# davxy/ark-vrf

Hardware: NVIDIA B200
Metric: bandersnatch_thin_vrf_batch_verified_proofs_per_sec (higher is better)
Workload: dtype u32

## Files before the change

__graft_entry__.py:

```python
import os
import subprocess
import sys

ROOT = os.path.dirname(os.path.abspath(__file__))
CSRC = os.path.join(ROOT, "ark_vrf_b200", "csrc")
LIB = os.path.join(ROOT, "ark_vrf_b200", "libavrf_gpu.so")
NVCC_FLAGS = ["-gencode", "arch=compute_100a,code=sm_100a", "-O3", "-lineinfo", "-std=c++17",
              "-Xcompiler", "-fPIC", "-shared"]


def _newer(target, sources):
    if not os.path.exists(target):
        return False
    t = os.path.getmtime(target)
    return all(os.path.getmtime(s) <= t for s in sources)


def build() -> None:
    srcs = [os.path.join(CSRC, f) for f in sorted(os.listdir(CSRC)) if f.endswith((".cu", ".cuh", ".h", ".cpp", ".inl"))]
    srcs.append(os.path.join(ROOT, "include", "avrf.h"))
    if not _newer(LIB, srcs):
        nvcc = os.environ.get("NVCC", "/usr/local/cuda/bin/nvcc")
        tmp = LIB + ".tmp"
        cmd = [nvcc] + NVCC_FLAGS + ["-o", tmp, os.path.join(CSRC, "avrf_gpu.cu"), os.path.join(CSRC, "mbsha512.cpp"),
                                   os.path.join(CSRC, "hostutil.cpp"),
                                   "-lcrypto", "-lpthread"]
        print("[build]", " ".join(cmd), flush=True)
        if os.path.exists(LIB):
            os.remove(LIB)
        subprocess.check_call(cmd)
        os.replace(tmp, LIB)
    emu_src = os.path.join(ROOT, "tests", "hostemu", "hostemu.cpp")
    emu_lib = os.path.join(ROOT, "tests", "hostemu", "libhostemu.so")
    if not _newer(emu_lib, srcs + [emu_src]):
        subprocess.check_call(["g++", "-O2", "-shared", "-fPIC", "-Wno-unknown-pragmas", "-o", emu_lib, emu_src])
    pl_src = os.path.join(ROOT, "tools", "push_loop.cpp")
    pl_lib = os.path.join(ROOT, "tools", "libavrf_pushloop.so")
    hdrs = [os.path.join(ROOT, "include", "avrf.h"), os.path.join(ROOT, "include", "avrf.hpp")]
    if os.path.exists(pl_src) and not _newer(pl_lib, hdrs + [pl_src, LIB]):
        pkg = os.path.join(ROOT, "ark_vrf_b200")
        subprocess.check_call(["g++", "-std=c++17", "-O2", "-shared", "-fPIC", "-I", os.path.join(ROOT, "include"), pl_src,
                               "-o", pl_lib, "-L", pkg, "-l:libavrf_gpu.so", "-Wl,-rpath," + pkg])
    mk = os.path.join(ROOT, "oracle", "Makefile")
    if os.path.exists(mk):
        subprocess.check_call(["make", "-s", "-C", os.path.join(ROOT, "oracle")])
    sys.path.insert(0, ROOT)
    import ark_vrf_b200
    ark_vrf_b200.load()


def smoke() -> None:
    sys.path.insert(0, ROOT)
    sys.path.insert(0, os.path.join(ROOT, "tests"))
    import ark_vrf_b200 as av
    from ark_vrf_b200 import synth
    from oracle import pyref as o
    av.load().avrf_init(0)
    sid, S, n = 0, o.BANDERSNATCH, 64
# ... 27 lines not shown
```

ark_vrf_b200/csrc/avrf_gpu.cu:

```cuda
#include <cstdlib>
#include <map>
#include <memory>
#include <new>
#include <vector>

#include "host_common.h"
#include "hostutil.h"
#include "feeders.cuh"
#include "verify_one.cuh"
#include "microbench.cuh"

using namespace avrf;

constexpr size_t PREP_CHUNK = 148 * 4 * 128;
constexpr size_t STAGE_CHUNK = PREP_CHUNK / 2;

struct PushStage {
  PinBuf pk, r, s, ios, ad, io_off, ad_off;
  size_t n = 0, nio = 0, nad = 0, cap_io = 0, cap_ad = 0;
  cudaEvent_t free_ev = nullptr;
  bool inflight = false;
};

struct avrf_batch {
  int device = 0;
  uint32_t suite = 0, fmt = 0, weights_mode = AVRF_WEIGHTS_REFERENCE;
  uint32_t scheme = 0;
  uint64_t n = 0, n_ios = 0, ad_bytes = 0;
  bool prepared = false;
  bool have_seed = false;
  bool want_taps = false;
  uint8_t seed[64];
  uint64_t first_index = 0;
  std::vector<uint64_t> segs;
  bool segs_dirty = false;
  DevBuf pk, r, s, ios, io_off, ad_off, ad;
  DevBuf ok, sb;
  PushStage stage[2];
  int cur = 0;
  std::vector<uint8_t> h_pk, h_r, h_s, h_ios, h_ad;
  std::vector<uint32_t> h_io_off{0}, h_ad_off{0};
  DevBuf dig_w, rank_w;
  DevBuf pts, cs, z, renc, digits, hist, cursor, offs, toff, btot, totals, entries, tasks, task_out, chunk_out, wsum,
      partial, gpart, flags, w_tap, scalars_tap, segs_dev;
  PinBuf h_cs, h_small;
  std::vector<cudaEvent_t> prep_ev;
  size_t prep_ev_chunks = 0;
  bool eager = true;
  std::unique_ptr<Hasher> hasher;
  Hasher* ext_hasher = nullptr;
  MbSha512* mb = nullptr;
  bool blocking = false;
  cudaEvent_t sync_ev = nullptr;
  uint64_t hashed = 0;
  uint64_t push_launches = 0;
  cudaStream_t st = nullptr, st_copy = nullptr, st_h2d = nullptr, st_prep = nullptr;
  ShardSlot* remote_slot = nullptr;
  bool inflight = false;
  bool inflight_did_prepare = false;
  int32_t early_status = -1;
  cudaEvent_t done_ev = nullptr;
  cudaEvent_t gate_ev = nullptr;
  cudaEvent_t h2d_gate_ev = nullptr;
  std::chrono::steady_clock::time_point t_verify0;
  cudaEvent_t ev[10] = {};
  avrf_timings tm = {};
};
// ... 30 lines not shown
  return CC_HOST[suite].suite_id;
}

static int finish_inflight(avrf_batch* b);

static int enter(avrf_batch* b) {
  if (!b) return fail(AVRF_ERR_ARG, "null batch");
  int rc = bind_device(b->device);
  if (rc) return rc;
  return b->inflight ? finish_inflight(b) : 0;
}
#define ENTER(b) do { int rc__ = enter(b); if (rc__) return rc__; } while (0)

static int quiesce(avrf_batch* b) {
  for (cudaStream_t q : {b->st_h2d, b->st_prep, b->st_copy, b->st}) CK(hsync(b, q));
  return 0;
}
static int grow(avrf_batch* b, DevBuf& buf, size_t bytes, size_t keep) {
  if (bytes <= buf.cap) return 0;
  int rc = quiesce(b);
  return rc ? rc : buf.reserve(bytes, keep, b->st);
}

static Hasher* hasher_of(avrf_batch* b) {
  if (b->ext_hasher) return b->ext_hasher;
  if (!b->hasher) {
    b->hasher.reset(new (std::nothrow) Hasher(b->device));
    if (b->hasher && b->mb) b->hasher->use_multibuffer(b->mb);
  }
  return b->hasher.get();
}

struct H2cScratch { DevBuf u01, den, scr; };
struct FeedPool {
  std::mutex mu;
  DevBuf b[12];
  H2cScratch w;
};
static FeedPool g_feed[AVRF_MAX_DEV];
static void feed_pool_release(int dev) {
  FeedPool& fp = g_feed[dev];
  std::lock_guard<std::mutex> lk(fp.mu);
  for (DevBuf& d : fp.b) d.release();
  fp.w.u01.release(); fp.w.den.release(); fp.w.scr.release();
}

// ... 114 lines not shown
  if (!b) return;
  bind_device(b->device);
  if (b->inflight) finish_inflight(b);
  b->hasher.reset();
  if (b->done_ev) cudaEventDestroy(b->done_ev);
  if (b->gate_ev) {
    MsmGate& g = g_gate[b->device];
    std::lock_guard<std::mutex> lk(g.mu);
    if (g.tail == b->gate_ev) g.tail = nullptr;
    cudaStreamSynchronize(b->st);
    cudaEventDestroy(b->gate_ev);
  }
  if (b->h2d_gate_ev) {
    MsmGate& g = g_h2d_gate[b->device];
    std::lock_guard<std::mutex> lk(g.mu);
    if (g.tail == b->h2d_gate_ev) g.tail = nullptr;
    cudaStreamSynchronize(b->st_h2d);
    cudaEventDestroy(b->h2d_gate_ev);
  }
  for (cudaStream_t q : {b->st, b->st_copy, b->st_h2d, b->st_prep}) if (q) cudaStreamSynchronize(q);
  DevBuf* bufs[] = {&b->ok, &b->sb, &b->pk, &b->r, &b->s, &b->ios, &b->io_off, &b->ad_off, &b->ad, &b->pts, &b->cs, &b->z, &b->renc,
                    &b->dig_w, &b->rank_w, &b->digits, &b->hist, &b->cursor, &b->offs, &b->toff, &b->btot, &b->totals, &b->entries, &b->tasks,
                    &b->task_out, &b->chunk_out, &b->wsum, &b->partial, &b->gpart, &b->flags, &b->w_tap, &b->scalars_tap,
                    &b->segs_dev};
  for (DevBuf* d : bufs) d->release();
  for (auto& e : b->ev) if (e) cudaEventDestroy(e);
  for (auto& e : b->prep_ev) cudaEventDestroy(e);
  for (auto& sg : b->stage) if (sg.free_ev) cudaEventDestroy(sg.free_ev);
  if (b->sync_ev) cudaEventDestroy(b->sync_ev);
  for (cudaStream_t q : {b->st, b->st_copy, b->st_h2d, b->st_prep}) if (q) cudaStreamDestroy(q);
  delete b;
}

int avrf_thin_batch_clear(avrf_batch* b) {
  ENTER(b);
  if (b->hasher) b->hasher->drain();
  for (auto& sg : b->stage) {
    if (sg.inflight) { CK(cudaEventSynchronize(sg.free_ev)); sg.inflight = false; }
    sg.n = sg.nio = sg.nad = 0;
  }
  b->n = b->n_ios = b->ad_bytes = 0;
  b->prepared = b->have_seed = false;
  b->hashed = 0;
  b->push_launches = 0;
  b->prep_ev_chunks = 0;
  b->segs.clear();
  b->segs_dirty = true;
// ... 166 lines not shown
      CK(cudaMemcpyAsync(b->sb.as<uint8_t>() + 32 * n0, sb, 32 * n, cudaMemcpyHostToDevice, b->st));
    }
    if (add_ios) CK(cudaMemcpyAsync(b->ios.as<uint8_t>() + 128 * i0, ios, 128 * add_ios, cudaMemcpyDefault, b->st));
    if (add_ad) CK(cudaMemcpyAsync(b->ad.as<uint8_t>() + a0, ad_blob, add_ad, cudaMemcpyDefault, b->st));
    if (consumed) CK(cudaEventRecord(consumed, b->st));
    b->n += n;
    b->n_ios += add_ios;
    b->ad_bytes += add_ad;
    b->prepared = b->have_seed = false;
    b->hashed = 0;
    b->prep_ev_chunks = 0;
    return 0;
  }
  Hasher* hs = hasher_of(b);
  if (!hs) return fail(AVRF_ERR_NOMEM, "hasher");
  size_t np_new = ped ? 5 * (n0 + n) + 2 : 2 * (n0 + n) + 2 * (i0 + add_ios) + 1;
  size_t np_old = n0 ? (ped ? 5 * n0 : 2 * n0 + 2 * i0) : 0;
  if ((rc = b->flags.reserve(64))) return rc;
  if ((rc = b->h_small.reserve(4096))) return rc;
  if ((rc = grow(b, b->pts, sizeof(BaseRec) * np_new, sizeof(BaseRec) * np_old))) return rc;
  if ((rc = grow(b, b->cs, stride * (n0 + n) + 64, stride * n0))) return rc;
  if ((rc = grow(b, b->z, 16 * (i0 + add_ios) + 16, 16 * i0))) return rc;
  if ((rc = grow(b, b->renc, 32 * (n0 + n) + 32, 32 * n0))) return rc;
  if (n0 == 0) {
    if (!b->ext_hasher) {
      size_t sl;
      const unsigned char* sid = suite_id_of(b->suite, &sl);
      unsigned char prefix[40];
      memcpy(prefix, sid, sl);
      prefix[sl] = DOM_BATCH;
      if ((rc = hs->begin(prefix, sl + 1))) return rc;
    }
    CK(cudaMemsetAsync(b->flags.p, 0, 64, b->st_prep));
  }
  if ((rc = hs->reserve_stage(std::max(stride * std::min<size_t>(n, 16 * PREP_CHUNK) + 64, stage_chunks * (stride * PREP_CHUNK + 64))))) return rc;
  size_t nch = (n + PREP_CHUNK - 1) / PREP_CHUNK;
  EventPool evs;
  cudaEvent_t off_ev = evs.make();
  if (!off_ev) return fail(AVRF_ERR_CUDA, "cudaEventCreate");
  CK(cudaEventRecord(off_ev, b->st_prep));
  CK(cudaStreamWaitEvent(b->st_h2d, off_ev, 0));
  PrepArgs a;
  PedPrepArgs pa;
  if (ped) {
    pa.pkcom = b->pk.as<Affine>(); pa.r = b->r.as<Affine>(); pa.ok = b->ok.as<Affine>(); pa.s = b->s.as<Fe>();
    pa.sb = b->sb.as<Fe>(); pa.ios = b->ios.as<Affine>(); pa.io_off = b->io_off.as<uint32_t>();
// ... 20 lines not shown
    CK(cudaMemcpyAsync(b->pk.as<uint8_t>() + 64 * (n0 + c0), pk + 64 * c0, 64 * cnt, cudaMemcpyDefault, b->st_h2d));
    CK(cudaMemcpyAsync(b->r.as<uint8_t>() + 64 * (n0 + c0), r + 64 * c0, 64 * cnt, cudaMemcpyDefault, b->st_h2d));
    CK(cudaMemcpyAsync(b->s.as<uint8_t>() + 32 * (n0 + c0), s + 32 * c0, 32 * cnt, cudaMemcpyDefault, b->st_h2d));
    if (ped) {
      CK(cudaMemcpyAsync(b->ok.as<uint8_t>() + 64 * (n0 + c0), ok + 64 * c0, 64 * cnt, cudaMemcpyDefault, b->st_h2d));
      CK(cudaMemcpyAsync(b->sb.as<uint8_t>() + 32 * (n0 + c0), sb + 32 * c0, 32 * cnt, cudaMemcpyDefault, b->st_h2d));
    }
    if (q1 > q0) CK(cudaMemcpyAsync(b->ios.as<uint8_t>() + 128 * (i0 + q0), ios + 128 * q0, 128 * (q1 - q0), cudaMemcpyDefault, b->st_h2d));
    if (d1 > d0) CK(cudaMemcpyAsync(b->ad.as<uint8_t>() + a0 + d0, ad_blob + d0, d1 - d0, cudaMemcpyDefault, b->st_h2d));
    CK(cudaEventRecord(h2d_ev, b->st_h2d));
    CK(cudaStreamWaitEvent(b->st_prep, h2d_ev, 0));
    if (ped) {
      pa.first = (uint32_t)(n0 + c0);
      pa.n = (uint32_t)(n0 + c1);
      DISPATCH(b->suite, (k_prepare_ped<S><<<cdiv(cnt, 128), 128, 0, b->st_prep>>>(pa)));
    } else {
      a.first = (uint32_t)(n0 + c0);
      a.n = (uint32_t)(n0 + c1);
      DISPATCH(b->suite, (k_prepare<S><<<cdiv(cnt, 128), 128, 0, b->st_prep>>>(a)));
    }
    LAUNCHED("k_prepare");
    CK(cudaEventRecord(prep_ev, b->st_prep));
    CK(cudaStreamWaitEvent(b->st_copy, prep_ev, 0));
    uint8_t* dst = hs->stage(stride * cnt);
    if (!dst) return fail(AVRF_ERR_NOMEM, "pinned staging");
    CK(cudaMemcpyAsync(dst, b->cs.as<uint8_t>() + stride * (n0 + c0), stride * cnt, cudaMemcpyDeviceToHost, b->st_copy));
    CK(cudaEventCreateWithFlags(&d2h_ev, cudaEventDisableTiming | cudaEventBlockingSync));
    CK(cudaEventRecord(d2h_ev, b->st_copy));
    hs->enqueue(d2h_ev, dst, stride * cnt);
  }
  CK(cudaEventRecord(b->h2d_gate_ev, b->st_h2d));
  hgate.tail = b->h2d_gate_ev;
  hgate_lock.unlock();
  if (consumed) CK(cudaEventRecord(consumed, b->st_prep));
  b->n += n;
  b->n_ios += add_ios;
  b->ad_bytes += add_ad;
  b->hashed = b->n;
  b->prepared = true;
  b->have_seed = false;
  b->prep_ev_chunks = 0;
  b->push_launches += nch;
  return 0;
}

static int stage_reserve(PushStage& sg, size_t cap_io, size_t cap_ad) {
  int rc;
  if ((rc = sg.pk.reserve(64 * PREP_CHUNK)) || (rc = sg.r.reserve(64 * PREP_CHUNK)) || (rc = sg.s.reserve(32 * PREP_CHUNK)) ||
      (rc = sg.io_off.reserve(4 * (PREP_CHUNK + 1))) || (rc = sg.ad_off.reserve(4 * (PREP_CHUNK + 1))))
    return rc;
  if (cap_io > sg.cap_io) { if ((rc = sg.ios.reserve(128 * cap_io, 128 * sg.nio))) return rc; sg.cap_io = cap_io; }
  if (cap_ad > sg.cap_ad) { if ((rc = sg.ad.reserve(cap_ad, sg.nad))) return rc; sg.cap_ad = cap_ad; }
  if (!sg.free_ev) CK(cudaEventCreateWithFlags(&sg.free_ev, cudaEventDisableTiming));
  return 0;
}

static int flush_stage(avrf_batch* b) {
  PushStage& sg = b->stage[b->cur];
  if (sg.n == 0) return 0;
  { int rc0 = bind_device(b->device); if (rc0) return rc0; }
  stage_fence();
  int rc = push_many_impl(b, sg.n, sg.pk.as<uint8_t>(), sg.ios.as<uint8_t>(), sg.io_off.as<uint32_t>(), sg.ad.as<uint8_t>(),
                          sg.ad_off.as<uint32_t>(), sg.r.as<uint8_t>(), sg.s.as<uint8_t>(), nullptr, nullptr, sg.free_ev,
                          sg.n == STAGE_CHUNK ? 4 : 0);
  if (rc) return rc;
// ... 71 lines not shown
  if ((io_offsets[n] && !ios) || (ad_offsets[n] && !ad_blob)) return fail(AVRF_ERR_ARG, "null argument");
  ENTER(b);
  int rc = flush_pending(b);
  if (rc) return rc;
  rc = push_many_impl(b, n, pk, ios, io_offsets, ad_blob, ad_offsets, r, s);
  if (rc) return rc;
  CK(hsync(b, b->st_h2d));
  CK(hsync(b, b->prepared ? b->st_prep : b->st));
  return 0;
}

int avrf_thin_batch_prepare(avrf_batch* b, int32_t* invalid) {
  ENTER(b);
  int rc = flush_pending(b);
  if (rc) return rc;
  if ((rc = b->flags.reserve(64))) return rc;
  if ((rc = b->h_small.reserve(4096))) return rc;
  if (!b->prepared) {
    size_t np = npoints_of(b);
    if ((rc = grow(b, b->pts, sizeof(BaseRec) * np, 0))) return rc;
    if ((rc = grow(b, b->cs, cs_stride(b) * b->n + 64, 0))) return rc;
    if ((rc = grow(b, b->z, 16 * b->n_ios + 16, 0))) return rc;
    if ((rc = grow(b, b->renc, 32 * b->n + 32, 0))) return rc;
    CK(cudaMemsetAsync(b->flags.p, 0, 64, b->st));
    size_t nch = (b->n + PREP_CHUNK - 1) / PREP_CHUNK;
    while (b->prep_ev.size() < nch) {
      cudaEvent_t e;
      CK(cudaEventCreateWithFlags(&e, cudaEventDisableTiming));
      b->prep_ev.push_back(e);
    }
    PedPrepArgs pa;
    PrepArgs ta;
    if (b->scheme == 1) {
      pa.pkcom = b->pk.as<Affine>(); pa.r = b->r.as<Affine>(); pa.ok = b->ok.as<Affine>(); pa.s = b->s.as<Fe>();
      pa.sb = b->sb.as<Fe>(); pa.ios = b->ios.as<Affine>(); pa.io_off = b->io_off.as<uint32_t>();
      pa.ad_off = b->ad_off.as<uint32_t>(); pa.ad = b->ad.as<uint8_t>(); pa.pts = b->pts.as<BaseRec>();
      pa.cs = b->cs.as<uint32_t>(); pa.flags = b->flags.as<int>(); pa.n = (uint32_t)b->n;
      pa.canonical = b->fmt == AVRF_FMT_CANONICAL;
    } else {
      ta.pk = b->pk.as<Affine>(); ta.r = b->r.as<Affine>(); ta.s = b->s.as<Fe>(); ta.ios = b->ios.as<Affine>();
      ta.io_off = b->io_off.as<uint32_t>(); ta.ad_off = b->ad_off.as<uint32_t>(); ta.ad = b->ad.as<uint8_t>();
      ta.pts = b->pts.as<BaseRec>(); ta.cs = b->cs.as<uint32_t>(); ta.z = b->z.as<uint32_t>();
      ta.renc = b->renc.as<uint32_t>(); ta.flags = b->flags.as<int>(); ta.n = (uint32_t)b->n;
      ta.canonical = b->fmt == AVRF_FMT_CANONICAL;
    }
    cudaStream_t ps = b->st_prep;
    {
      cudaEvent_t e;
      CK(cudaEventCreateWithFlags(&e, cudaEventDisableTiming));
      cudaEventRecord(e, b->st);
      cudaStreamWaitEvent(ps, e, 0);
      cudaEventDestroy(e);
    }
    if (nch) cudaEventRecord(b->ev[0], ps);
    for (size_t c = 0; c < nch; c++) {
      size_t cnt = std::min((size_t)PREP_CHUNK, (size_t)b->n - c * PREP_CHUNK);
      if (b->scheme == 1) {
        pa.first = (uint32_t)(c * PREP_CHUNK);
        DISPATCH(b->suite, (k_prepare_ped<S><<<cdiv(cnt, 128), 128, 0, ps>>>(pa)));
      } else {
        ta.first = (uint32_t)(c * PREP_CHUNK);
        DISPATCH(b->suite, (k_prepare<S><<<cdiv(cnt, 128), 128, 0, ps>>>(ta)));
      }
      LAUNCHED(b->scheme == 1 ? "k_prepare_ped" : "k_prepare");
      CK(cudaEventRecord(b->prep_ev[c], ps));
    }
    if (nch) {
      cudaEventRecord(b->ev[1], ps);
      cudaStreamWaitEvent(b->st, b->ev[1], 0);
      b->tm.kernel_launches = nch;
    }
    b->prep_ev_chunks = nch;
    b->prepared = true;
    b->have_seed = false;
  } else {
    cudaEvent_t e;
    CK(cudaEventCreateWithFlags(&e, cudaEventDisableTiming));
    cudaEventRecord(e, b->st_prep);
    cudaStreamWaitEvent(b->st, e, 0);
    cudaEventDestroy(e);
  }
  if (invalid) {
    CK(cudaMemcpyAsync(b->h_small.p, b->flags.p, 8, cudaMemcpyDeviceToHost, b->st));
    CK(hsync(b, b->st));
    int fl = reinterpret_cast<int*>(b->h_small.p)[0];
    if (fl & 2) return fail(AVRF_ERR_ARG, "an input coordinate or scalar is not below its modulus (not a field element)");
    *invalid = fl & 1;
  }
  return 0;
}

int avrf_thin_batch_cs_stream(avrf_batch* b, uint8_t* out) {
  if (!b || !out) return fail(AVRF_ERR_ARG, "null argument");
// ... 156 lines not shown
  if (b->want_taps) {
    if ((rc = b->w_tap.reserve(32 * b->n + 32))) return rc;
    if ((rc = b->scalars_tap.reserve(32 * np))) return rc;
  }
  cudaStream_t st = b->st;
  if (!b->gate_ev) CK(cudaEventCreateWithFlags(&b->gate_ev, cudaEventDisableTiming));
  if (b->segs.size() > 2 && b->segs_dirty) {
    if ((rc = b->segs_dev.reserve(8 * b->segs.size()))) return rc;
    CK(cudaMemcpyAsync(b->segs_dev.p, b->segs.data(), 8 * b->segs.size(), cudaMemcpyHostToDevice, st));
    CK(hsync(b, st));
    b->segs_dirty = false;
  }
  MsmGate& gate = g_gate[b->device];
  std::unique_lock<std::mutex> gate_lock(gate.mu);
  if (gate.tail && gate.tail != b->gate_ev) CK(cudaStreamWaitEvent(st, gate.tail, 0));
  CK(cudaMemsetAsync(b->hist.p, 0, 4 * MSM_NBINS, st));

  ScalArgs a;
  a.cs = b->cs.as<uint32_t>(); a.z = b->z.as<uint32_t>(); a.io_off = b->io_off.as<uint32_t>();
  a.digits = b->digits.as<uint4>(); a.hist = b->hist.as<uint32_t>(); a.gpart = b->gpart.as<uint32_t>();
  a.ranks = b->cursor.as<uint4>();
  a.w_tap = b->want_taps ? b->w_tap.as<uint32_t>() : nullptr;
  a.scalars_tap = b->want_taps ? b->scalars_tap.as<Fe>() : nullptr;
  seed_to_words(a.seed, seed);
  a.first_index = b->segs.size() == 2 ? b->segs[1] : first_index;
  a.segs = b->segs.size() > 2 ? b->segs_dev.as<uint64_t>() : nullptr;
  a.nseg = (uint32_t)(b->segs.size() / 2);
  b->first_index = first_index;
  a.n = (uint32_t)b->n;
  uint32_t* hist = b->hist.as<uint32_t>();
  uint32_t* offs = b->offs.as<uint32_t>();
  uint32_t* nzr = b->toff.as<uint32_t>();
  uint32_t* totals = b->totals.as<uint32_t>();
  Ext* slots = b->task_out.as<Ext>();
  cudaEventRecord(b->ev[2], st);
  if (b->scheme == 1) {
    PedScalArgs pa;
    pa.cs = a.cs; pa.digits = a.digits; pa.ranks = a.ranks; pa.hist = a.hist; pa.gpart = a.gpart;
    pa.w_tap = b->want_taps ? b->w_tap.as<uint32_t>() : nullptr;
    pa.scalars_tap = a.scalars_tap; pa.seed = a.seed; pa.first_index = a.first_index; pa.segs = a.segs; pa.nseg = a.nseg;
    pa.n = a.n;
    DISPATCH(b->suite, (k_scalars_ped<S><<<nblk, 128, 0, st>>>(pa)));
    LAUNCHED("k_scalars_ped");
    DISPATCH(b->suite, (k_gscalar_ped<S><<<1, 32, 0, st>>>(a.gpart, nblk, a.digits, a.ranks, a.hist, a.scalars_tap,
                                                            b->pts.as<BaseRec>(), np - 2)));
    LAUNCHED("k_gscalar_ped");
  } else {
    DISPATCH(b->suite, (k_scalars<S><<<nblk, 128, 0, st>>>(a)));
    LAUNCHED("k_scalars");
    DISPATCH(b->suite, (k_gscalar<S><<<1, 256, 0, st>>>(a.gpart, nblk, a.digits, a.ranks, a.hist, a.scalars_tap,
                                                         b->pts.as<BaseRec>(), np - 1)));
    LAUNCHED("k_gscalar");
  }
  cudaEventRecord(b->ev[3], st);
  k_scan_local<<<MSM_NBINS / 1024, 1024, 0, st>>>(hist, offs, nzr, b->btot.as<uint32_t>());
  LAUNCHED("k_scan_local");
  k_scan_totals<<<1, 512, 0, st>>>(b->btot.as<uint32_t>(), totals, offs);
  LAUNCHED("k_scan_totals");
  k_scan_add<<<MSM_NBINS / 1024, 1024, 0, st>>>(offs, nzr, b->btot.as<uint32_t>());
  LAUNCHED("k_scan_add");
  if (np >= (1u << 18)) {
    static std::once_flag smem_once[AVRF_MAX_DEV];
    std::call_once(smem_once[b->device], [] {
      cudaFuncSetAttribute(k_scatter_window, cudaFuncAttributeMaxDynamicSharedMemorySize, 4 * MSM_NBUCKET);
    });
    k_sort_transpose<<<cdiv(np, SORT_TP), SORT_TP, 0, st>>>(b->digits.as<uint4>(), b->cursor.as<uint4>(), np, np_pad,
                                                            b->dig_w.as<uint16_t>(), b->rank_w.as<uint32_t>());
    LAUNCHED("k_sort_transpose");
    k_scatter_window<<<dim3(37, MSM_NWIN), 1024, 4 * MSM_NBUCKET, st>>>(b->dig_w.as<uint16_t>(), b->rank_w.as<uint32_t>(), np, np_pad,
                                                                         offs, b->entries.as<uint32_t>());
    LAUNCHED("k_scatter_window");
  } else {
// ... 7 lines not shown
  ac.pts = b->pts.as<BaseRec>(); ac.slots = slots; ac.nthr = acc_nthr;
  if (b->suite == 0) k_accumulate<0, 4><<<acc_blocks, 128, 0, st>>>(ac);
  else if (b->suite == 2) k_accumulate<2, 4><<<acc_blocks, 128, 0, st>>>(ac);
  else k_accumulate<1, 5><<<acc_blocks, 128, 0, st>>>(ac);
  LAUNCHED("k_accumulate");
  cudaEventRecord(b->ev[5], st);
  CK(cudaEventRecord(b->gate_ev, st));
  gate.tail = b->gate_ev;
  gate_lock.unlock();
  DISPATCH(b->suite, (k_combine<S><<<MSM_NBINS / 128, 128, 0, st>>>(hist, offs, nzr, slots, acc_nthr, totals,
                                                                    b->tasks.as<uint32_t>())));
  LAUNCHED("k_combine");
  DISPATCH(b->suite, (k_combine_big<S><<<64, 256, 0, st>>>(hist, offs, nzr, slots, acc_nthr, totals,
                                                           b->tasks.as<uint32_t>())));
  LAUNCHED("k_combine_big");
  DISPATCH(b->suite, (k_bucket_reduce<S><<<MSM_NWIN * MSM_NCHUNK / 128, 128, 0, st>>>(hist, offs, nzr, acc_nthr, totals, slots,
                                                                                      b->chunk_out.as<Ext>())));
  LAUNCHED("k_bucket_reduce");
  DISPATCH(b->suite, (k_window_sum<S><<<MSM_NWIN, 256, 0, st>>>(b->chunk_out.as<Ext>(), b->wsum.as<Ext>())));
  LAUNCHED("k_window_sum");
  DISPATCH(b->suite, (k_fold<S><<<1, 32, 0, st>>>(b->wsum.as<Ext>(), b->partial.as<Ext>(), b->flags.as<int>(), b->remote_slot)));
  LAUNCHED("k_fold");
  cudaEventRecord(b->ev[6], st);
  b->tm.kernel_launches += 12;
  b->tm.n_points = np;
  return 0;
}

static void collect_timings(avrf_batch* b, bool with_prepare) {
  float ms = 0;
  if (with_prepare && cudaEventElapsedTime(&ms, b->ev[0], b->ev[1]) == cudaSuccess) b->tm.prepare_ms = ms;
  if (cudaEventElapsedTime(&ms, b->ev[2], b->ev[3]) == cudaSuccess) b->tm.scalars_ms = ms;
  if (cudaEventElapsedTime(&ms, b->ev[3], b->ev[4]) == cudaSuccess) b->tm.sort_ms = ms;
  if (cudaEventElapsedTime(&ms, b->ev[4], b->ev[5]) == cudaSuccess) b->tm.accumulate_ms = ms;
  if (cudaEventElapsedTime(&ms, b->ev[5], b->ev[6]) == cudaSuccess) b->tm.reduce_ms = ms;
  (void)cudaGetLastError();
}

extern "C" {

int avrf_thin_seed_dev(uint32_t suite, const void* cs_stream_dev, uint64_t n_items, uint8_t seed[64]) {
  if (suite > 2 || !seed || (n_items && !cs_stream_dev)) return fail(AVRF_ERR_ARG, "bad argument");
  NEED_DEVICE();
  std::lock_guard<std::mutex> lock(g_pin_mu);
  return seed_of_device_stream(gs(), gc(), suite, (const uint8_t*)cs_stream_dev, 64 * n_items, g_pin_stream[g_device.load()], seed, nullptr);
}

// ... 264 lines not shown
```

ark_vrf_b200/csrc/msm.cuh:

```cuda
#pragma once
#include "thin.cuh"

namespace avrf {

constexpr int MSM_WBITS = 16;
constexpr int MSM_NWIN = 16;
constexpr int MSM_NBUCKET = 1 << (MSM_WBITS - 1);
constexpr int MSM_NBINS = MSM_NWIN * MSM_NBUCKET;
constexpr int MSM_CHUNK = 16;
constexpr int MSM_NCHUNK = MSM_NBUCKET / MSM_CHUNK;

struct Seed64 { uint64_t w[8]; };

#ifdef __CUDACC__

__device__ __forceinline__ void load_affinek(AffineK& q, const BaseRec* p) {
  const uint4* s = reinterpret_cast<const uint4*>(p);
  uint4 a0 = __ldg(s + 0), a1 = __ldg(s + 1), a2 = __ldg(s + 2), a3 = __ldg(s + 3), a4 = __ldg(s + 4), a5 = __ldg(s + 5);
  q.x.v[0] = a0.x; q.x.v[1] = a0.y; q.x.v[2] = a0.z; q.x.v[3] = a0.w;
  q.x.v[4] = a1.x; q.x.v[5] = a1.y; q.x.v[6] = a1.z; q.x.v[7] = a1.w;
  q.y.v[0] = a2.x; q.y.v[1] = a2.y; q.y.v[2] = a2.z; q.y.v[3] = a2.w;
  q.y.v[4] = a3.x; q.y.v[5] = a3.y; q.y.v[6] = a3.z; q.y.v[7] = a3.w;
  q.k.v[0] = a4.x; q.k.v[1] = a4.y; q.k.v[2] = a4.z; q.k.v[3] = a4.w;
  q.k.v[4] = a5.x; q.k.v[5] = a5.y; q.k.v[6] = a5.z; q.k.v[7] = a5.w;
// ... 1 lines not shown

__device__ __forceinline__ void store_fe(Fe* dst, const Fe& a) {
  uint4* d = reinterpret_cast<uint4*>(dst);
  d[0] = make_uint4(a.v[0], a.v[1], a.v[2], a.v[3]);
  d[1] = make_uint4(a.v[4], a.v[5], a.v[6], a.v[7]);
}

__device__ __forceinline__ void load_fe(Fe& a, const Fe* src) {
  const uint4* s = reinterpret_cast<const uint4*>(src);
  uint4 lo = s[0], hi = s[1];
  a.v[0] = lo.x; a.v[1] = lo.y; a.v[2] = lo.z; a.v[3] = lo.w;
  a.v[4] = hi.x; a.v[5] = hi.y; a.v[6] = hi.z; a.v[7] = hi.w;
}

__device__ __forceinline__ void store_ext(Ext* dst, const Ext& p) {
  store_fe(&dst->x, p.x); store_fe(&dst->y, p.y); store_fe(&dst->z, p.z); store_fe(&dst->t, p.t);
}

__device__ __forceinline__ void load_ext(Ext& p, const Ext* src) {
  load_fe(p.x, &src->x); load_fe(p.y, &src->y); load_fe(p.z, &src->z); load_fe(p.t, &src->t);
}

__device__ __forceinline__ void emit_scalar(uint4* digits, uint32_t* hist, uint4* ranks, Fe* scalars_tap, size_t point,
                                            const Fe& k) {
  int32_t dg[16];
  recode_signed16(dg, k);
  uint32_t pk[8];
#pragma unroll
  for (int i = 0; i < 8; i++) pk[i] = ((uint32_t)dg[2 * i] & 0xffffu) | ((uint32_t)dg[2 * i + 1] << 16);
  digits[2 * point] = make_uint4(pk[0], pk[1], pk[2], pk[3]);
  digits[2 * point + 1] = make_uint4(pk[4], pk[5], pk[6], pk[7]);
  uint32_t rk[16];
#pragma unroll
  for (int i = 0; i < 16; i++) {
    int32_t d = dg[i];
    rk[i] = 0;
    if (d != 0) {
      uint32_t mag = d < 0 ? (uint32_t)(-d) : (uint32_t)d;
      rk[i] = atomicAdd(&hist[i * MSM_NBUCKET + mag - 1], 1u);
    }
  }
#pragma unroll
  for (int i = 0; i < 4; i++) ranks[4 * point + i] = make_uint4(rk[4 * i], rk[4 * i + 1], rk[4 * i + 2], rk[4 * i + 3]);
  if (scalars_tap) store_fe(&scalars_tap[point], k);
}

struct ScalArgs {
  const uint32_t* cs;
  const uint32_t* z;
  const uint32_t* io_off;
  uint4* digits;
  uint4* ranks;
  uint32_t* hist;
  uint32_t* gpart;
  uint32_t* w_tap;
  Fe* scalars_tap;
  Seed64 seed;
  uint64_t first_index;
  const uint64_t* segs;
  uint32_t nseg;
  uint32_t n;
};

__device__ __forceinline__ uint64_t global_index(uint64_t first_index, const uint64_t* segs, uint32_t nseg, uint32_t j) {
  if (nseg <= 1) return first_index + j;
  uint32_t lo = 0, hi = nseg;
  while (hi - lo > 1) {
    uint32_t mid = (lo + hi) >> 1;
    if (segs[2 * mid] <= j) lo = mid;
    else hi = mid;
  }
  return segs[2 * lo + 1] + (j - segs[2 * lo]);
}

__device__ __forceinline__ void add10(uint32_t* a, const uint32_t* b) {
  a[0] = add_cc(a[0], b[0]);
#pragma unroll
  for (int i = 1; i < 9; i++) a[i] = addc_cc(a[i], b[i]);
  a[9] = addc(a[9], b[9]);
}

constexpr uint32_t SCAL_PER_THREAD = 1;
template <int S>
__global__ void __launch_bounds__(128) k_scalars(ScalArgs a) {
  constexpr int FR = SuiteT<S>::FR;
// ... 8 lines not shown
    if ((jg >> 2) != have) {
      have = jg >> 2;
      sha512_xof_block(blk, a.seed.w, have);
    }
    Fe w, c, s, wM, wc, ws;
    fe_zero(w);
    fe_zero(c);
    digest_le128(w.v, blk, 16 * (uint32_t)(jg & 3));
    const uint32_t* csj = a.cs + 16 * (size_t)j;
#pragma unroll
    for (int i = 0; i < 4; i++) c.v[i] = csj[i];
#pragma unroll
    for (int i = 0; i < 8; i++) s.v[i] = csj[8 + i];
    if (a.w_tap) {
#pragma unroll
      for (int i = 0; i < 4; i++) a.w_tap[4 * (size_t)j + i] = w.v[i];
    }
    to_mont<FR>(wM, w);
    mont_mul_c<FR>(wc, wM, c);
    mont_mul_c<FR>(ws, wM, s);
    uint32_t io0 = a.io_off[j], io1 = a.io_off[j + 1];
    size_t pbase = 2 * (size_t)j + 2 * (size_t)io0;
    emit_scalar(a.digits, a.hist, a.ranks, a.scalars_tap, pbase + 0, w);
    emit_scalar(a.digits, a.hist, a.ranks, a.scalars_tap, pbase + 1, wc);
    for (uint32_t i = io0; i < io1; i++) {
      Fe z, zM, t;
      fe_zero(z);
#pragma unroll
      for (int q = 0; q < 4; q++) z.v[q] = a.z[4 * (size_t)i + q];
      to_mont<FR>(zM, z);
      mont_mul_c<FR>(t, wc, zM);
      emit_scalar(a.digits, a.hist, a.ranks, a.scalars_tap, pbase + 2 + 2 * (size_t)(i - io0), t);
      mont_mul_c<FR>(t, ws, zM);
      fe_neg<FR>(t, t);
      emit_scalar(a.digits, a.hist, a.ranks, a.scalars_tap, pbase + 3 + 2 * (size_t)(i - io0), t);
    }
    uint32_t wsv[10];
#pragma unroll
    for (int i = 0; i < 8; i++) wsv[i] = ws.v[i];
    wsv[8] = wsv[9] = 0;
    add10(acc, wsv);
  }
#pragma unroll
  for (int off = 16; off > 0; off >>= 1) {
    uint32_t o[10];
#pragma unroll
    for (int i = 0; i < 10; i++) o[i] = __shfl_down_sync(0xffffffffu, acc[i], off);
    add10(acc, o);
  }
  __shared__ uint32_t sm[4][10];
  int warp = threadIdx.x >> 5, lane = threadIdx.x & 31;
  if (lane == 0) {
#pragma unroll
    for (int i = 0; i < 10; i++) sm[warp][i] = acc[i];
  }
  __syncthreads();
  if (threadIdx.x == 0) {
    for (int wv = 1; wv < 4; wv++) add10(acc, sm[wv]);
#pragma unroll
    for (int i = 0; i < 10; i++) a.gpart[10 * (size_t)blockIdx.x + i] = acc[i];
  }
}

template <int S>
__global__ void __launch_bounds__(256) k_gscalar(const uint32_t* gpart, uint32_t nblocks, uint4* digits, uint4* ranks,
                                                 uint32_t* hist, Fe* scalars_tap, BaseRec* pts, size_t gpoint) {
  constexpr int FR = SuiteT<S>::FR;
  __shared__ uint32_t sm[8][10];
  uint32_t acc[10];
#pragma unroll
  for (int i = 0; i < 10; i++) acc[i] = 0;
  for (uint32_t b = threadIdx.x; b < nblocks; b += blockDim.x) add10(acc, gpart + 10 * (size_t)b);
#pragma unroll
  for (int off = 16; off > 0; off >>= 1) {
    uint32_t o[10];
#pragma unroll
    for (int i = 0; i < 10; i++) o[i] = __shfl_down_sync(0xffffffffu, acc[i], off);
    add10(acc, o);
  }
  int warp = threadIdx.x >> 5, lane = threadIdx.x & 31;
  if (lane == 0) {
#pragma unroll
    for (int i = 0; i < 10; i++) sm[warp][i] = acc[i];
  }
// ... 615 lines not shown
```

ark_vrf_b200/csrc/prepare.cuh:

```cuda
#pragma once
#include "msm.cuh"

namespace avrf {
template <int F>
__device__ __forceinline__ bool fe_in_range(const Fe& a) { return limbs_gt(AVRF_FC(F).p, a.v); }

template <int S>
__device__ __forceinline__ void load_affine_fmt(Affine& p, const Affine* src, int canonical, int* oob = nullptr) {
  load_fe(p.x, &src->x);
  load_fe(p.y, &src->y);
  if (oob) *oob |= !(fe_in_range<SuiteT<S>::FQ>(p.x) && fe_in_range<SuiteT<S>::FQ>(p.y));
  if (canonical) {
    to_mont<SuiteT<S>::FQ>(p.x, p.x);
    to_mont<SuiteT<S>::FQ>(p.y, p.y);
  }
}

template <int S>
__device__ __forceinline__ void store_affine_fmt(Affine* dst, const Affine& p, int canonical) {
  Affine q = p;
  if (canonical) {
    from_mont<SuiteT<S>::FQ>(q.x, q.x);
    from_mont<SuiteT<S>::FQ>(q.y, q.y);
  }
// ... 63 lines not shown
  uint32_t* zout = a.z + 4 * (size_t)io0;
  thin_delinearize(t, m, [&](uint32_t i, const uint32_t* z4) {
    zout[4 * i + 0] = z4[0]; zout[4 * i + 1] = z4[1]; zout[4 * i + 2] = z4[2]; zout[4 * i + 3] = z4[3];
  });
  load_affine_fmt<S>(P, a.r + j, a.canonical, &oob);
  affine_compress<S>(enc, P);
  affine_to_k<S>(K, P);
  store_affinek(a.pts + pbase, K);
  uint32_t c4[4];
  thin_challenge(t, enc, c4);
  Fe s;
  load_fe(s, a.s + j);
  oob |= !fe_in_range<FR>(s);
  if (!a.canonical) from_mont<FR>(s, s);
  uint4* cs = reinterpret_cast<uint4*>(a.cs + 16 * (size_t)j);
  cs[0] = make_uint4(c4[0], c4[1], c4[2], c4[3]);
  cs[1] = make_uint4(0, 0, 0, 0);
  cs[2] = make_uint4(s.v[0], s.v[1], s.v[2], s.v[3]);
  cs[3] = make_uint4(s.v[4], s.v[5], s.v[6], s.v[7]);
  uint4* re = reinterpret_cast<uint4*>(a.renc + 8 * (size_t)j);
  re[0] = make_uint4(enc[0], enc[1], enc[2], enc[3]);
  re[1] = make_uint4(enc[4], enc[5], enc[6], enc[7]);
  if (bad | (oob != 0)) atomicOr(a.flags, (bad ? 1 : 0) | (oob ? 2 : 0));
}

constexpr uint32_t TREE_LEAF = 32;
__global__ void __launch_bounds__(64) k_tree_leaves(const uint32_t* cs, uint32_t n, uint64_t first_leaf, uint64_t* out) {
  uint32_t l = blockIdx.x * blockDim.x + threadIdx.x;
  uint32_t nl = (n + TREE_LEAF - 1) / TREE_LEAF;
  if (l >= nl) return;
  Sha512 c;
  sha512_init(c);
  sha512_put_byte(c, 0);
  sha512_put_le64(c, first_leaf + l);
  uint32_t j0 = l * TREE_LEAF, j1 = min(n, j0 + TREE_LEAF);
  for (uint32_t j = j0; j < j1; j++) {
    const uint32_t* w = cs + 16 * (size_t)j;
    sha512_put_words(c, w);
    sha512_put_words(c, w + 8);
  }
  uint64_t d[8];
  sha512_final(c, d);
  for (int i = 0; i < 8; i++) out[8 * (size_t)l + i] = bswap64(d[i]);
}

struct PedPrepArgs {
// ... 122 lines not shown
```

Before: 81.84 million.

## Deduplicate repeated public keys and merge their MSM scalars per key

Adds a GPU hash table, built during prepare, that groups proofs sharing the same public key, with an on-curve check for each group's representative. When computing scalars, proofs in a group of two or more add their key-point scalar into a per-group 64-bit-limb accumulator using warp-level match, shuffle and atomics, and zero their own digits. A new kernel then reduces each group sum modulo the cofactor-scaled group order and emits it on the representative point. The goal is less bucket-accumulation work in the MSM when signers repeat. The cost is extra kernels, memsets and atomics, which buy nothing if all keys in the batch are distinct.

```diff
diff --git a/__graft_entry__.py b/__graft_entry__.py
--- a/__graft_entry__.py
+++ b/__graft_entry__.py
@@ -34,6 +34,10 @@
     emu_lib = os.path.join(ROOT, "tests", "hostemu", "libhostemu.so")
     if not _newer(emu_lib, srcs + [emu_src]):
         subprocess.check_call(["g++", "-O2", "-shared", "-fPIC", "-Wno-unknown-pragmas", "-o", emu_lib, emu_src])
+    keys_src = os.path.join(ROOT, "tests", "hostemu", "keys_emu.cpp")
+    keys_lib = os.path.join(ROOT, "tests", "hostemu", "libkeysemu.so")
+    if not _newer(keys_lib, srcs + [keys_src]):
+        subprocess.check_call(["g++", "-O2", "-shared", "-fPIC", "-Wno-unknown-pragmas", "-o", keys_lib, keys_src])
     pl_src = os.path.join(ROOT, "tools", "push_loop.cpp")
     pl_lib = os.path.join(ROOT, "tools", "libavrf_pushloop.so")
     hdrs = [os.path.join(ROOT, "include", "avrf.h"), os.path.join(ROOT, "include", "avrf.hpp")]
diff --git a/ark_vrf_b200/csrc/avrf_gpu.cu b/ark_vrf_b200/csrc/avrf_gpu.cu
--- a/ark_vrf_b200/csrc/avrf_gpu.cu
+++ b/ark_vrf_b200/csrc/avrf_gpu.cu
@@ -43,6 +43,8 @@
   DevBuf dig_w, rank_w;
   DevBuf pts, cs, z, renc, digits, hist, cursor, offs, toff, btot, totals, entries, tasks, task_out, chunk_out, wsum,
       partial, gpart, flags, w_tap, scalars_tap, segs_dev;
+  DevBuf keys, grp;
+  size_t key_cap = 0;
   PinBuf h_cs, h_small;
   std::vector<cudaEvent_t> prep_ev;
   size_t prep_ev_chunks = 0;
@@ -119,6 +121,40 @@
   return rc ? rc : buf.reserve(bytes, keep, b->st);
 }
 
+static unsigned long long* key_acc(avrf_batch* b) { return b->keys.as<unsigned long long>(); }
+static uint32_t* key_slot(avrf_batch* b) { return reinterpret_cast<uint32_t*>(key_acc(b) + 8 * b->key_cap); }
+static uint32_t* key_cnt(avrf_batch* b) { return key_slot(b) + b->key_cap; }
+static size_t key_cap_for(uint64_t n) {
+  size_t cap = 1024;
+  while (cap < 2 * n) cap <<= 1;
+  return cap;
+}
+
+static int keys_reset(avrf_batch* b, uint64_t n, cudaStream_t st) {
+  int rc;
+  if ((rc = grow(b, b->grp, 4 * n + 4, 0))) return rc;
+  size_t cap = key_cap_for(n);
+  if (cap > b->key_cap) {
+    if ((rc = grow(b, b->keys, 72 * cap, 0))) return rc;
+    b->key_cap = cap;
+    CK(cudaMemsetAsync(b->keys.p, 0, 64 * cap, st));
+  }
+  CK(cudaMemsetAsync(key_slot(b), 0xff, 4 * b->key_cap, st));
+  CK(cudaMemsetAsync(key_cnt(b), 0, 4 * b->key_cap, st));
+  return 0;
+}
+
+static int keys_insert(avrf_batch* b, uint64_t first, uint64_t n, cudaStream_t st) {
+  if (n <= first) return 0;
+  KeyArgs k;
+  k.pk = b->pk.as<uint4>(); k.slot = key_slot(b); k.cnt = key_cnt(b); k.grp = b->grp.as<uint32_t>();
+  k.mask = (uint32_t)(b->key_cap - 1); k.first = (uint32_t)first; k.n = (uint32_t)n;
+  k.canonical = b->fmt == AVRF_FMT_CANONICAL;
+  DISPATCH(b->suite, (k_key_insert<S><<<cdiv(n - first, 128), 128, 0, st>>>(k)));
+  LAUNCHED("k_key_insert");
+  return 0;
+}
+
 static Hasher* hasher_of(avrf_batch* b) {
   if (b->ext_hasher) return b->ext_hasher;
   if (!b->hasher) {
@@ -279,7 +315,7 @@
   DevBuf* bufs[] = {&b->ok, &b->sb, &b->pk, &b->r, &b->s, &b->ios, &b->io_off, &b->ad_off, &b->ad, &b->pts, &b->cs, &b->z, &b->renc,
                     &b->dig_w, &b->rank_w, &b->digits, &b->hist, &b->cursor, &b->offs, &b->toff, &b->btot, &b->totals, &b->entries, &b->tasks,
                     &b->task_out, &b->chunk_out, &b->wsum, &b->partial, &b->gpart, &b->flags, &b->w_tap, &b->scalars_tap,
-                    &b->segs_dev};
+                    &b->segs_dev, &b->keys, &b->grp};
   for (DevBuf* d : bufs) d->release();
   for (auto& e : b->ev) if (e) cudaEventDestroy(e);
   for (auto& e : b->prep_ev) cudaEventDestroy(e);
@@ -492,6 +528,13 @@
   if ((rc = grow(b, b->cs, stride * (n0 + n) + 64, stride * n0))) return rc;
   if ((rc = grow(b, b->z, 16 * (i0 + add_ios) + 16, 16 * i0))) return rc;
   if ((rc = grow(b, b->renc, 32 * (n0 + n) + 32, 32 * n0))) return rc;
+  if (!ped) {
+    if (n0 == 0 || key_cap_for(n0 + n) > b->key_cap) {
+      if ((rc = keys_reset(b, n0 + n, b->st_prep)) || (rc = keys_insert(b, 0, n0, b->st_prep))) return rc;
+    } else if ((rc = grow(b, b->grp, 4 * (n0 + n) + 4, 4 * n0))) {
+      return rc;
+    }
+  }
   if (n0 == 0) {
     if (!b->ext_hasher) {
       size_t sl;
@@ -558,6 +601,7 @@
     LAUNCHED("k_prepare");
     CK(cudaEventRecord(prep_ev, b->st_prep));
     CK(cudaStreamWaitEvent(b->st_copy, prep_ev, 0));
+    if (!ped && (rc = keys_insert(b, n0 + c0, n0 + c1, b->st_prep))) return rc;
     uint8_t* dst = hs->stage(stride * cnt);
     if (!dst) return fail(AVRF_ERR_NOMEM, "pinned staging");
     CK(cudaMemcpyAsync(dst, b->cs.as<uint8_t>() + stride * (n0 + c0), stride * cnt, cudaMemcpyDeviceToHost, b->st_copy));
@@ -576,7 +620,7 @@
   b->prepared = true;
   b->have_seed = false;
   b->prep_ev_chunks = 0;
-  b->push_launches += nch;
+  b->push_launches += ped ? nch : 2 * nch;
   return 0;
 }
 
@@ -694,6 +738,7 @@
     if ((rc = grow(b, b->cs, cs_stride(b) * b->n + 64, 0))) return rc;
     if ((rc = grow(b, b->z, 16 * b->n_ios + 16, 0))) return rc;
     if ((rc = grow(b, b->renc, 32 * b->n + 32, 0))) return rc;
+    if (b->scheme == 0 && (rc = keys_reset(b, b->n, b->st))) return rc;
     CK(cudaMemsetAsync(b->flags.p, 0, 64, b->st));
     size_t nch = (b->n + PREP_CHUNK - 1) / PREP_CHUNK;
     while (b->prep_ev.size() < nch) {
@@ -737,10 +782,11 @@
       LAUNCHED(b->scheme == 1 ? "k_prepare_ped" : "k_prepare");
       CK(cudaEventRecord(b->prep_ev[c], ps));
     }
+    if (b->scheme == 0 && (rc = keys_insert(b, 0, b->n, ps))) return rc;
     if (nch) {
       cudaEventRecord(b->ev[1], ps);
       cudaStreamWaitEvent(b->st, b->ev[1], 0);
-      b->tm.kernel_launches = nch;
+      b->tm.kernel_launches = nch + (b->scheme == 0);
     }
     b->prep_ev_chunks = nch;
     b->prepared = true;
@@ -943,6 +989,7 @@
   a.ranks = b->cursor.as<uint4>();
   a.w_tap = b->want_taps ? b->w_tap.as<uint32_t>() : nullptr;
   a.scalars_tap = b->want_taps ? b->scalars_tap.as<Fe>() : nullptr;
+  a.grp = b->key_cap ? b->grp.as<uint32_t>() : nullptr; a.kcnt = key_cnt(b); a.kacc = key_acc(b);
   seed_to_words(a.seed, seed);
   a.first_index = b->segs.size() == 2 ? b->segs[1] : first_index;
   a.segs = b->segs.size() > 2 ? b->segs_dev.as<uint64_t>() : nullptr;
@@ -969,6 +1016,12 @@
   } else {
     DISPATCH(b->suite, (k_scalars<S><<<nblk, 128, 0, st>>>(a)));
     LAUNCHED("k_scalars");
+    if (b->key_cap) {
+      DISPATCH(b->suite, (k_key_scalars<S><<<cdiv(b->key_cap, 256), 256, 0, st>>>(key_slot(b), key_cnt(b), key_acc(b),
+                                                                                    (uint32_t)b->key_cap, a.io_off, a.digits,
+                                                                                    a.ranks, a.hist)));
+      LAUNCHED("k_key_scalars");
+    }
     DISPATCH(b->suite, (k_gscalar<S><<<1, 256, 0, st>>>(a.gpart, nblk, a.digits, a.ranks, a.hist, a.scalars_tap,
                                                          b->pts.as<BaseRec>(), np - 1)));
     LAUNCHED("k_gscalar");
@@ -1022,7 +1075,7 @@
   DISPATCH(b->suite, (k_fold<S><<<1, 32, 0, st>>>(b->wsum.as<Ext>(), b->partial.as<Ext>(), b->flags.as<int>(), b->remote_slot)));
   LAUNCHED("k_fold");
   cudaEventRecord(b->ev[6], st);
-  b->tm.kernel_launches += 12;
+  b->tm.kernel_launches += b->scheme ? 12 : 13;
   b->tm.n_points = np;
   return 0;
 }
diff --git a/ark_vrf_b200/csrc/keys.cuh b/ark_vrf_b200/csrc/keys.cuh
--- /dev/null
+++ b/ark_vrf_b200/csrc/keys.cuh
@@ -0,0 +1,114 @@
+#pragma once
+#include "curve.cuh"
+
+namespace avrf {
+
+constexpr uint32_t KEY_EMPTY = 0xffffffffu;
+constexpr uint32_t KEY_NOGROUP = 0x80000000u;
+
+AVRF_HD uint32_t key_hash(const uint32_t* w) {
+  uint32_t h = 0x9e3779b9u;
+#pragma unroll
+  for (int i = 0; i < 16; i++) {
+    h = (h ^ w[i]) * 0x85ebca6bu;
+    h ^= h >> 13;
+  }
+  h *= 0xc2b2ae35u;
+  return h ^ (h >> 16);
+}
+
+AVRF_HD void key_sum_normalise(uint32_t* x, const uint64_t* acc) {
+  uint64_t carry = 0;
+#pragma unroll
+  for (int i = 0; i < 8; i++) {
+    uint64_t t = acc[i] + carry;
+    x[i] = (uint32_t)t;
+    carry = t >> 32;
+  }
+  x[8] = (uint32_t)carry;
+}
+
+AVRF_HD void key_reduce(uint32_t* k, const uint32_t* x9, const uint32_t* m) {
+  uint32_t x[10];
+#pragma unroll
+  for (int i = 0; i < 9; i++) x[i] = x9[i];
+  x[9] = 0;
+#pragma unroll 1
+  for (int sh = 35; sh >= 0; sh--) {
+    uint32_t t[10];
+    const int ws = sh >> 5, bs = sh & 31;
+    for (int i = 0; i < 10; i++) {
+      int s = i - ws;
+      uint32_t lo = s >= 0 && s < 8 ? m[s] : 0u;
+      uint32_t below = s - 1 >= 0 && s - 1 < 8 ? m[s - 1] : 0u;
+      t[i] = bs ? (lo << bs) | (below >> (32 - bs)) : lo;
+    }
+    bool ge = true;
+    for (int i = 9; i >= 0; i--)
+      if (x[i] != t[i]) { ge = x[i] > t[i]; break; }
+    if (!ge) continue;
+    uint64_t borrow = 0;
+    for (int i = 0; i < 10; i++) {
+      uint64_t d = (uint64_t)x[i] - t[i] - borrow;
+      x[i] = (uint32_t)d;
+      borrow = (d >> 32) & 1u;
+    }
+  }
+#pragma unroll
+  for (int i = 0; i < 8; i++) k[i] = x[i];
+}
+
+template <int S>
+AVRF_HD void key_group_order(uint32_t* m) {
+  const uint32_t* r = AVRF_FC(SuiteT<S>::FR).p;
+  const uint32_t c = AVRF_CC(S).cof_log2;
+#pragma unroll
+  for (int i = 7; i > 0; i--) m[i] = (r[i] << c) | (r[i - 1] >> (32 - c));
+  m[0] = r[0] << c;
+}
+
+template <int S>
+AVRF_HD void key_sum_scalar(Fe& k, bool* neg, const uint64_t* acc) {
+  uint32_t x[9], m[8];
+  key_sum_normalise(x, acc);
+  key_group_order<S>(m);
+  key_reduce(k.v, x, m);
+  *neg = k.v[7] >= 0x40000000u;
+  if (*neg) {
+    uint64_t borrow = 0;
+#pragma unroll
+    for (int i = 0; i < 8; i++) {
+      uint64_t d = (uint64_t)m[i] - k.v[i] - borrow;
+      k.v[i] = (uint32_t)d;
+      borrow = (d >> 32) & 1u;
+    }
+  }
+}
+
+AVRF_HD void recode_signed16_neg(int32_t* dg, const Fe& k) {
+  uint32_t carry = 0;
+#pragma unroll
+  for (int i = 0; i < 16; i++) {
+    uint32_t v = ((k.v[i >> 1] >> (16 * (i & 1))) & 0xffffu) + carry;
+    if (v > 32768u) { dg[i] = 65536 - (int32_t)v; carry = 1; }
+    else { dg[i] = -(int32_t)v; carry = 0; }
+  }
+}
+
+template <int S>
+AVRF_HD bool affine_on_curve(const Affine& P) {
+  constexpr int FQ = SuiteT<S>::FQ;
+  Fe x2, y2, t, u, one, d;
+  mont_sqr_c<FQ>(x2, P.x);
+  mont_sqr_c<FQ>(y2, P.y);
+  fe_set(d, AVRF_CC(S).d);
+  fe_one<FQ>(one);
+  mont_mul_c<FQ>(t, x2, y2);
+  mont_mul_c<FQ>(t, t, d);
+  fe_add<FQ>(t, t, one);
+  fe_sub<FQ>(t, t, y2);
+  sub_a_times<S>(u, t, x2);
+  return fe_is_zero(u);
+}
+
+}
diff --git a/ark_vrf_b200/csrc/msm.cuh b/ark_vrf_b200/csrc/msm.cuh
--- a/ark_vrf_b200/csrc/msm.cuh
+++ b/ark_vrf_b200/csrc/msm.cuh
@@ -1,5 +1,6 @@
 #pragma once
 #include "thin.cuh"
+#include "keys.cuh"
 
 namespace avrf {
 
@@ -47,9 +48,10 @@
 }
 
 __device__ __forceinline__ void emit_scalar(uint4* digits, uint32_t* hist, uint4* ranks, Fe* scalars_tap, size_t point,
-                                            const Fe& k) {
+                                            const Fe& k, bool neg = false) {
   int32_t dg[16];
-  recode_signed16(dg, k);
+  if (neg) recode_signed16_neg(dg, k);
+  else recode_signed16(dg, k);
   uint32_t pk[8];
 #pragma unroll
   for (int i = 0; i < 8; i++) pk[i] = ((uint32_t)dg[2 * i] & 0xffffu) | ((uint32_t)dg[2 * i + 1] << 16);
@@ -80,12 +82,37 @@
   uint32_t* gpart;
   uint32_t* w_tap;
   Fe* scalars_tap;
+  const uint32_t* grp;
+  const uint32_t* kcnt;
+  unsigned long long* kacc;
   Seed64 seed;
   uint64_t first_index;
   const uint64_t* segs;
   uint32_t nseg;
   uint32_t n;
 };
+
+__device__ __forceinline__ void key_accumulate(unsigned long long* kacc, uint32_t g, const Fe& wc) {
+  const uint32_t m = __match_any_sync(__activemask(), g);
+  const uint32_t lane = threadIdx.x & 31;
+  unsigned long long s[8];
+#pragma unroll
+  for (int i = 0; i < 8; i++) s[i] = wc.v[i];
+  if (m != (1u << lane)) {
+#pragma unroll
+    for (int i = 0; i < 8; i++) s[i] = 0;
+#pragma unroll 1
+    for (uint32_t r = m; r; r &= r - 1) {
+      const int src = __ffs(r) - 1;
+#pragma unroll
+      for (int i = 0; i < 8; i++) s[i] += __shfl_sync(m, wc.v[i], src);
+    }
+  }
+  if (lane == (uint32_t)(__ffs(m) - 1)) {
+#pragma unroll
+    for (int i = 0; i < 8; i++) atomicAdd(&kacc[8 * (size_t)g + i], s[i]);
+  }
+}
 
 __device__ __forceinline__ uint64_t global_index(uint64_t first_index, const uint64_t* segs, uint32_t nseg, uint32_t j) {
   if (nseg <= 1) return first_index + j;
@@ -140,7 +167,15 @@
     uint32_t io0 = a.io_off[j], io1 = a.io_off[j + 1];
     size_t pbase = 2 * (size_t)j + 2 * (size_t)io0;
     emit_scalar(a.digits, a.hist, a.ranks, a.scalars_tap, pbase + 0, w);
-    emit_scalar(a.digits, a.hist, a.ranks, a.scalars_tap, pbase + 1, wc);
+    uint32_t g = a.grp ? a.grp[j] : 0u, gc = a.grp ? a.kcnt[g] : 0u;
+    if (gc >= 2u && gc < KEY_NOGROUP) {
+      key_accumulate(a.kacc, g, wc);
+      a.digits[2 * (pbase + 1)] = make_uint4(0, 0, 0, 0);
+      a.digits[2 * (pbase + 1) + 1] = make_uint4(0, 0, 0, 0);
+      if (a.scalars_tap) store_fe(&a.scalars_tap[pbase + 1], wc);
+    } else {
+      emit_scalar(a.digits, a.hist, a.ranks, a.scalars_tap, pbase + 1, wc);
+    }
     for (uint32_t i = io0; i < io1; i++) {
       Fe z, zM, t;
       fe_zero(z);
@@ -178,6 +213,31 @@
 #pragma unroll
     for (int i = 0; i < 10; i++) a.gpart[10 * (size_t)blockIdx.x + i] = acc[i];
   }
+}
+
+template <int S>
+__global__ void __launch_bounds__(256) k_key_scalars(const uint32_t* __restrict__ kslot, const uint32_t* __restrict__ kcnt,
+                                                     unsigned long long* __restrict__ kacc, uint32_t cap,
+                                                     const uint32_t* __restrict__ io_off, uint4* digits, uint4* ranks,
+                                                     uint32_t* hist) {
+  uint32_t s = blockIdx.x * blockDim.x + threadIdx.x;
+  if (s >= cap) return;
+  uint32_t c = kcnt[s];
+  if (c < 2u || c >= KEY_NOGROUP) return;
+  uint32_t rep = kslot[s];
+  uint64_t acc[8];
+  ulonglong2* p = reinterpret_cast<ulonglong2*>(kacc + 8 * (size_t)s);
+#pragma unroll
+  for (int i = 0; i < 4; i++) {
+    ulonglong2 v = p[i];
+    acc[2 * i] = v.x;
+    acc[2 * i + 1] = v.y;
+    p[i] = make_ulonglong2(0, 0);
+  }
+  Fe k;
+  bool neg;
+  key_sum_scalar<S>(k, &neg, acc);
+  emit_scalar(digits, hist, ranks, nullptr, 2 * (size_t)rep + 2 * (size_t)io_off[rep] + 1, k, neg);
 }
 
 template <int S>
diff --git a/ark_vrf_b200/csrc/prepare.cuh b/ark_vrf_b200/csrc/prepare.cuh
--- a/ark_vrf_b200/csrc/prepare.cuh
+++ b/ark_vrf_b200/csrc/prepare.cuh
@@ -109,6 +109,53 @@
   re[0] = make_uint4(enc[0], enc[1], enc[2], enc[3]);
   re[1] = make_uint4(enc[4], enc[5], enc[6], enc[7]);
   if (bad | (oob != 0)) atomicOr(a.flags, (bad ? 1 : 0) | (oob ? 2 : 0));
+}
+
+struct KeyArgs {
+  const uint4* pk;
+  uint32_t* slot;
+  uint32_t* cnt;
+  uint32_t* grp;
+  uint32_t mask;
+  uint32_t first, n;
+  int canonical;
+};
+
+template <int S>
+__global__ void __launch_bounds__(128) k_key_insert(KeyArgs a) {
+  uint32_t j = a.first + blockIdx.x * blockDim.x + threadIdx.x;
+  if (j >= a.n) return;
+  uint4 q[4];
+  uint32_t w[16];
+#pragma unroll
+  for (int i = 0; i < 4; i++) {
+    q[i] = __ldg(a.pk + 4 * (size_t)j + i);
+    w[4 * i] = q[i].x; w[4 * i + 1] = q[i].y; w[4 * i + 2] = q[i].z; w[4 * i + 3] = q[i].w;
+  }
+  uint32_t h = key_hash(w) & a.mask;
+#pragma unroll 1
+  for (;;) {
+    uint32_t rep = __ldcg(a.slot + h);
+    if (rep == KEY_EMPTY) {
+      rep = atomicCAS(a.slot + h, KEY_EMPTY, j);
+      if (rep == KEY_EMPTY) {
+        Affine P;
+        load_affine_fmt<S>(P, reinterpret_cast<const Affine*>(a.pk) + j, a.canonical);
+        if (!affine_on_curve<S>(P)) atomicOr(a.cnt + h, KEY_NOGROUP);
+        break;
+      }
+    }
+    bool same = true;
+#pragma unroll
+    for (int i = 0; i < 4; i++) {
+      uint4 r = __ldg(a.pk + 4 * (size_t)rep + i);
+      same &= r.x == q[i].x && r.y == q[i].y && r.z == q[i].z && r.w == q[i].w;
+    }
+    if (same) break;
+    h = (h + 1) & a.mask;
+  }
+  a.grp[j] = h;
+  atomicAdd(a.cnt + h, 1u);
 }
 
 constexpr uint32_t TREE_LEAF = 32;
```

Measured after the change: 91.05 million (median of 6 runs). +11.3%, better.
